# Vegeta2020/SE-SSD

Measured on NVIDIA H100. Metric: frames_per_sec, higher is better.
Workload: dtype f32

## Files before the change

include/sessd_b200.h:

```cpp
#ifndef SESSD_B200_H
#define SESSD_B200_H

#include <stddef.h>
#include <stdint.h>

#ifdef __cplusplus
extern "C" {
#endif

#define SESSD_OK 0
#define SESSD_EINVAL (-1)
#define SESSD_ECAPACITY (-2)
#define SESSD_EWORKSPACE (-3)

const char *sessd_version(void);
long long sessd_launch_count(void);

typedef struct {
    float voxel_size[3];
    float range_min[3];
    float range_max[3];
    int grid[3];
    int max_points;
    int max_voxels;
// ... 27 lines not shown

int sessd_strided_rulebook(const int *d_in_coors, const int *d_n_in, int max_in, sessd_grid in_grid,
                           int in_index_kind, const void *d_in_index, int in_hash_capacity,
                           const int ksize[3], const int stride[3], const int padding[3],
                           sessd_grid out_grid, void *d_out_bitmap , void *d_scan_scratch,
                           int *d_out_coors, int *d_n_out, int max_out, int *d_nbr, int *d_status, void *stream);

int sessd_tile_list_stride(int kvol);
int sessd_rulebook_tile_lists(const int *d_nbr, int kvol, const int *d_n_out, int max_out, void *d_tiles, void *stream);
size_t sessd_rulebook_pairs_workspace_bytes(int max_rows, int kvol);
int sessd_rulebook_pairs(const int *d_nbr, const int *d_n_out, int max_rows, int kvol, int *d_pairs_in,
                         int *d_pairs_out, int *d_pair_num, void *workspace, size_t workspace_bytes, void *stream);

int sessd_spconv_forward(const float *d_in_feat, int cin, const int *d_nbr, int kvol, const int *d_n_out,
                         int max_out, const float *d_weight, int cout, const float *d_scale, const float *d_shift,
                         int relu, float *d_out_feat, void *stream);

int sessd_sparse_to_dense(const float *d_feat, const int *d_coors, const int *d_n, int max_rows, int channels,
                          sessd_grid grid, float *d_out, void *stream);
int sessd_sparse_to_dense_indexed(const float *d_feat, int max_rows, const void *d_bitmap_index, int channels, sessd_grid grid,
                                  float *d_out, void *stream);

int sessd_spconv_forward_rows(const float *d_in_feat, int cin, const int *d_nbr, int kvol, const int *d_n_out, int max_out,
                              const float *d_weight, int cout, const float *d_scale, const float *d_shift, int relu,
                              float *d_out_feat, float *d_amax_out, void *stream);
int sessd_spconv_forward_rows_planes(const float *d_in_feat, int cin, const int *d_nbr, int kvol, const int *d_n_out, int max_out,
                                     const float *d_weight, int cout, const float *d_scale, const float *d_shift, int relu,
                                     const float *d_amax_in, float gain, float shift_max, float *d_out_feat, void *d_out_planes, int cpo,
                                     float *d_out_info, void *stream);
int sessd_spconv_forward_cg(const void *d_in_planes, int cp, int plane_rows, const float *d_in_info, const void *d_tiles, int kvol,
                            const int *d_n_out, int max_out, const void *d_weight_h2, int cout, const float *d_scale, const float *d_shift,
                            int relu, float gain, float shift_max, float *d_out_f32, void *d_out_planes, float *d_out_info, void *stream);
void sessd_set_sp_cg_deep(int on);
int sessd_absmax_rows(const float *d_feat, const int *d_n, int max_rows, int channels, float *d_amax, void *stream);

int sessd_rulebook_transpose(const int *d_nbr, int kvol, const int *d_n_out, int max_out, int max_in, int *d_nbr_t, void *stream);
int sessd_sparse_split_planes(const float *d_x, const int *d_n, int max_rows, int channels, float *d_info, void *d_planes, int cp, void *stream);
int sessd_dense_grad_gather(const float *d_grad, const int *d_coors, const int *d_n, int max_rows, int channels, sessd_grid grid,
                            float *d_out, void *stream);
int sessd_spconv_wgrad_items(int max_out, int kvol);
size_t sessd_spconv_wgrad_workspace_bytes(int max_out, int kvol, int cin, int cout);
int sessd_spconv_wgrad_rows(const float *d_in_feat, int cin, const float *d_gout, int cout, const void *d_tiles, int kvol,
                            const int *d_n_out, int max_out, float *d_gw, void *d_ws, size_t ws_bytes, void *stream);
int sessd_spconv_wgrad_cg(const void *d_in_planes, int cp, const float *d_in_info, const void *d_g_planes, int cout, const float *d_g_info,
                          const void *d_tiles, int kvol, const int *d_n_out, int max_out, float *d_gw, void *d_ws, size_t ws_bytes,
                          void *stream);

typedef struct {
    int batch, in_h, in_w, cin;
    int out_h, out_w, cout;
    int grid_h, grid_w;
    int in_stride;
    int out_stride, out_off_y, out_off_x;
    int ntaps;
    int tap_dy[16], tap_dx[16];
    int relu;
} sessd_conv_desc;

int sessd_bev_conv_p2(const void *d_in_planes, const float *d_in_info, const void *d_weight_h2, int cout_pad, const float *d_scale,
                      const float *d_shift, const float *d_residual, const float *d_resid_info, float gain, float shift_max,
                      float *d_out_f32, void *d_out_planes, float *d_out_info, const sessd_conv_desc *desc, const int *d_items,
                      void *stream);
int sessd_bev_deconv_p2(const void *d_in_planes, const float *d_in_info, const void *d_weight_h2, int cout_pad, const float *d_scale,
                        const float *d_shift, const float *d_residual, const float *d_resid_info, float gain, float shift_max,
                        float *d_out_f32, void *d_out_planes, float *d_out_info, int batch, int in_h, int in_w, int cin, int cout,
                        int relu, const int *d_items, void *stream);
// ... 169 lines not shown
```

se-ssd_b200/csrc/spconv_cg.cu:

```cuda
#include <cuda_fp16.h>

#include "tc_common.cuh"
#include "tile_lists.cuh"

namespace sessd {

constexpr int kCgBM = 128;
constexpr int kCgMaxK = 27;
constexpr int kCgProdWarps = 8;
constexpr int kCgMmaWarps = 8;
constexpr int kCgWeightWarp = kCgProdWarps + kCgMmaWarps;
constexpr int kCgThreads = (kCgWeightWarp + 1) * 32;

template <int CP, int COUT, int DEEP = 0>
struct CgCfg {
    static constexpr bool kWide = (CP == 64);
    static constexpr int kATile = (kWide ? 2 : 1) * kCgBM * 128;
    static constexpr int kBTile = (kWide ? 2 : 1) * COUT * 128;
    static constexpr int kStage = kATile + (kBTile + 1023) / 1024 * 1024;
    static constexpr int kStages = (kWide ? 2 : 4) * (DEEP ? 2 : 1);
    static constexpr int kMeta = kCgBM * kCgMaxK * 4  + kCgMaxK * 16  + 2 * COUT * 4  + 32 * 4  +
                                 33 * 4  + 32 * 4  + 3 * kStages * 8  + 24;
    static constexpr int kSmem = kStages * kStage + kMeta + 1024;
    static constexpr int kCPO = COUT > 32 ? 64 : 32;
};

struct CgArgs {
    const __half *planes;
    const float *in_info;
    const unsigned int *tiles;
    int tile_stride;
    const int *d_n_out;
    int kvol, max_out, relu;
    const float *scale, *shift;
    float gain, shift_max;
    float *out_f32;
    __half *out_planes;
    float *out_info;
};

__device__ __forceinline__ void cg_cp_async16(uint32_t smem_dst, const void *gsrc) {
    asm volatile("cp.async.cg.shared.global [%0], [%1], 16;\n" ::"r"(smem_dst), "l"(gsrc) : "memory");
}
__device__ __forceinline__ void cg_fence_proxy_async() { asm volatile("fence.proxy.async.shared::cta;\n" ::: "memory"); }
__device__ __forceinline__ void cg_sts_zero16(uint32_t saddr) {
    asm volatile("st.shared.v4.b32 [%0], {%1, %1, %1, %1};\n" ::"r"(saddr), "r"(0) : "memory");
}

template <int N>
__device__ __forceinline__ void cg_wgmma(float *d, uint64_t da, uint64_t db, uint32_t accumulate) {
    if constexpr (N == 32) wgmma_f16_n32(d, da, db, accumulate);
    else if constexpr (N == 64) wgmma_f16_n64(d, da, db, accumulate);
    else wgmma_f16_n128(d, da, db, accumulate);
}

template <int CP, int COUT, int DEEP>
__global__ void __launch_bounds__(kCgThreads, 1) spconv_cg_kernel(const __grid_constant__ CUtensorMap map_w, const CgArgs a) {
    using C = CgCfg<CP, COUT, DEEP>;
    const int n_out = min(*a.d_n_out, a.max_out);
    const int ntiles = (n_out + kCgBM - 1) / kCgBM;
    if ((int)blockIdx.x >= ntiles) return;
    const int kvol = a.kvol;
    if (threadIdx.x == kCgWeightWarp * 32) prefetch_tensormap(&map_w);

    extern __shared__ unsigned char smem_raw[];
    unsigned char *tiles = (unsigned char *)(((uintptr_t)smem_raw + 1023) & ~(uintptr_t)1023);
    uint32_t *s_list = (uint32_t *)(tiles + C::kStages * C::kStage);
    uint32_t *s_valid = s_list + kCgBM * kCgMaxK;
    float *s_scale = (float *)(s_valid + kCgMaxK * 4);
    float *s_shift = s_scale + COUT;
    int *s_cnt = (int *)(s_shift + COUT);
    int *s_klist = s_cnt + 32;
    int *s_nact = s_klist + 32;
    int *s_off = s_nact + 1;
    uint64_t *bars = (uint64_t *)(((uintptr_t)(s_off + 32) + 7) & ~(uintptr_t)7);
    uint64_t *full_a = bars, *full_b = bars + C::kStages, *empty = bars + 2 * C::kStages;

    const int tid = threadIdx.x, warp = tid >> 5, lane = tid & 31;
    const uint32_t tiles_u32 = smem_u32(tiles);

    if (tid == 0) {
        for (int s = 0; s < C::kStages; ++s) { mbar_init(&full_a[s], kCgProdWarps / C::kStages); mbar_init(&full_b[s], 1); mbar_init(&empty[s], kCgMmaWarps); }
        asm volatile("fence.mbarrier_init.release.cluster;\n" ::: "memory");
    }
    if (tid < COUT) {
        s_scale[tid] = __ldg(a.scale + tid);
        s_shift[tid] = a.shift ? __ldg(a.shift + tid) : 0.f;
    }
    for (int s = 0; s < C::kStages; ++s)
        for (int o = tid * 16; o < C::kATile; o += kCgThreads * 16) cg_sts_zero16(tiles_u32 + (uint32_t)(s * C::kStage + o));
    cg_fence_proxy_async();
    __syncthreads();

    const float amax_in = __ldg(a.in_info), s_in = __ldg(a.in_info + 1);
    const float inv_act = 1.f / s_in;
    const float s_out = pow2_scale_for_bound(amax_in * a.gain + a.shift_max);
    if (blockIdx.x == 0 && tid == 0 && a.out_info) a.out_info[1] = s_out;
    float vmax = 0.f;
    uint32_t dirty[4] = {0u, 0u, 0u, 0u};
    int st0 = 0;
    uint32_t ph0 = 0;

    for (int tile = blockIdx.x; tile < ntiles; tile += gridDim.x) {
        const int row0 = tile * kCgBM;
        const int rows = min(kCgBM, n_out - row0);
        {
            const unsigned int *rec = a.tiles + (size_t)tile * (size_t)a.tile_stride;
            const int c = (int)__ldg(rec + lane);
            unsigned int spec[4];
#pragma unroll
            for (int u = 0; u < 4; ++u) spec[u] = (tid + u * kCgThreads < kTlRows * kvol) ? __ldg(rec + kTlHeader + tid + u * kCgThreads) : 0u;
            const int incl = warp_incl_scan(c, lane);
            const int total = __shfl_sync(0xffffffffu, incl, 31);
            if (warp == 0) {
                s_cnt[lane] = c;
                s_off[lane] = incl - c;
                const unsigned int m = __ballot_sync(0xffffffffu, c > 0);
                if (c > 0) s_klist[__popc(m & ((1u << lane) - 1u))] = lane;
                if (lane == 0) *s_nact = __popc(m);
            }
            if (tid < kvol * 4) s_valid[tid] = __ldg(rec + kTlMask + tid);
#pragma unroll
            for (int u = 0; u < 4; ++u)
                if (tid + u * kCgThreads < total) s_list[tid + u * kCgThreads] = spec[u];
            for (int e = tid + 4 * kCgThreads; e < total; e += kCgThreads) s_list[e] = __ldg(rec + kTlHeader + e);
        }
        __syncthreads();
        const int nact = *s_nact;

        if (warp == kCgWeightWarp) {
            int s = st0;
            uint32_t ph = ph0;
            for (int j = 0; j < nact; ++j) {
                const int k = s_klist[j];
                mbar_wait(&empty[s], ph ^ 1u);
                if (elect_one()) {
                    mbar_expect_tx(&full_b[s], C::kBTile);
                    unsigned char *b_tile = tiles + s * C::kStage + C::kATile;
                    tma_load_4d(b_tile + C::kBTile / 2, &map_w, &full_b[s], 0, 0, 0, k);
                    tma_load_4d(b_tile, &map_w, &full_b[s], 0, 0, 1, k);
                }
                __syncwarp();
                if (++s == C::kStages) { s = 0; ph ^= 1u; }
            }
        } else if (warp >= kCgProdWarps) {
            const int cw = warp - kCgProdWarps, wg = cw >> 2, wq = cw & 3;
            constexpr int kAcc = COUT / 2;
            float acc[COUT];
#pragma unroll
            for (int i = 0; i < COUT; ++i) acc[i] = 0.f;
            const uint32_t a_rows = (uint32_t)(wg * 64 * 128);
            int s = st0;
            uint32_t ph = ph0;
            for (int j = 0; j < nact; ++j) {
                mbar_wait(&full_b[s], ph);
                mbar_wait(&full_a[s], ph);
                const uint32_t st = tiles_u32 + (uint32_t)(s * C::kStage);
                const uint64_t dA = kDescSw128Hi | desc_lo(st + a_rows);
                const uint32_t first = j != 0 ? 1u : 0u;
                wgmma_fence();
                if constexpr (C::kWide) {
                    const uint64_t dAl = dA + ((kCgBM * 128) >> 4);
                    const uint64_t dBl = kDescSw128Hi | desc_lo(st + C::kATile);
                    const uint64_t dBh = dBl + ((COUT * 128) >> 4);
#pragma unroll
                    for (int kk = 0; kk < 4; ++kk) cg_wgmma<2 * COUT>(acc, dA + 2 * kk, dBl + 2 * kk, first | (kk != 0));
#pragma unroll
                    for (int kk = 0; kk < 4; ++kk) cg_wgmma<COUT>(acc, dAl + 2 * kk, dBh + 2 * kk, 1u);
                } else {
                    const uint64_t dBl = kDescSw64Hi | desc_lo(st + C::kATile);
                    const uint64_t dBh = dBl + ((COUT * 64) >> 4);
#pragma unroll
                    for (int kk = 0; kk < 2; ++kk) cg_wgmma<2 * COUT>(acc, dA + 2 * kk, dBl + 2 * kk, first | (kk != 0));
#pragma unroll
                    for (int kk = 0; kk < 2; ++kk) cg_wgmma<COUT>(acc, dA + 4 + 2 * kk, dBh + 2 * kk, 1u);
                }
                wgmma_commit();
                wgmma_wait<0>();
                if (lane == 0) mbar_arrive(&empty[s]);
                if (++s == C::kStages) { s = 0; ph ^= 1u; }
            }
            wgmma_fence_regs<COUT>(acc);
#pragma unroll
            for (int i = 0; i < kAcc; ++i) acc[i] = acc[kAcc + i] + acc[i];
            const int q = lane & 3;
            const int r0 = wg * 64 + wq * 16 + (lane >> 2);
#pragma unroll
            for (int jb = 0; jb < COUT / 32; ++jb)
#pragma unroll
                for (int h = 0; h < 2; ++h) {
                    const int r = r0 + 8 * h;
                    const bool row_ok = r < rows;
                    const size_t orow = (size_t)(row0 + r);
                    float v[8], o[8];
                    quad_transpose8(acc + 16 * jb + 2 * h, q, v);
                    const int n = 32 * jb + 8 * q;
#pragma unroll
                    for (int t = 0; t < 8; t += 4) {
                        const float4 sc = *reinterpret_cast<const float4 *>(s_scale + n + t);
                        const float4 sh = *reinterpret_cast<const float4 *>(s_shift + n + t);
                        o[t] = fmaf(v[t] * inv_act, sc.x, sh.x);
                        o[t + 1] = fmaf(v[t + 1] * inv_act, sc.y, sh.y);
                        o[t + 2] = fmaf(v[t + 2] * inv_act, sc.z, sh.z);
                        o[t + 3] = fmaf(v[t + 3] * inv_act, sc.w, sh.w);
                    }
                    if (a.relu) {
#pragma unroll
                        for (int t = 0; t < 8; ++t) o[t] = fmaxf(o[t], 0.f);
                    }
                    if (row_ok) {
#pragma unroll
                        for (int t = 0; t < 8; ++t) vmax = fmaxf(vmax, fabsf(o[t]));
                    }
                    if (a.out_planes && row_ok) {
                        __align__(16) __half2 hi[4], lo[4];
#pragma unroll
                        for (int t = 0; t < 4; ++t) {
                            const float x0 = o[2 * t] * s_out, x1 = o[2 * t + 1] * s_out;
                            hi[t] = __floats2half2_rn(x0, x1);
                            const float2 f = __half22float2(hi[t]);
                            lo[t] = __floats2half2_rn(x0 - f.x, x1 - f.y);
                        }
                        __half *dst = a.out_planes + orow * (2 * C::kCPO) + n;
                        *reinterpret_cast<uint4 *>(dst) = *reinterpret_cast<const uint4 *>(hi);
                        *reinterpret_cast<uint4 *>(dst + C::kCPO) = *reinterpret_cast<const uint4 *>(lo);
                    }
                    if (a.out_f32) {
                        const bool up = q & 2;
                        float keep[4], recv[4];
#pragma unroll
                        for (int t = 0; t < 4; ++t) {
                            keep[t] = up ? o[4 + t] : o[t];
                            recv[t] = __shfl_xor_sync(0xFFFFFFFFu, up ? o[t] : o[4 + t], 2);
                        }
                        const float4 w_lo = up ? make_float4(recv[0], recv[1], recv[2], recv[3]) : make_float4(keep[0], keep[1], keep[2], keep[3]);
                        const float4 w_hi = up ? make_float4(keep[0], keep[1], keep[2], keep[3]) : make_float4(recv[0], recv[1], recv[2], recv[3]);
                        float *dst = a.out_f32 + orow * COUT + 32 * jb + 8 * (q & 1) + 4 * (q >> 1);
                        if (row_ok) {
                            *reinterpret_cast<float4 *>(dst) = w_lo;
                            *reinterpret_cast<float4 *>(dst + 16) = w_hi;
                        }
                    }
                }
        } else {
            constexpr int kGroupWarps = kCgProdWarps / C::kStages;
            constexpr int kGroupThreads = kGroupWarps * 32;
            constexpr int kOwnRows = kCgBM / kGroupWarps;
            constexpr int kOwnWords = kOwnRows / 32;
            constexpr int kLanesPerRow = C::kWide ? 16 : 8;
            constexpr int kRowsPerPass = kGroupThreads / kLanesPerRow;
            const int grp = warp / kGroupWarps, gw = warp % kGroupWarps;
            const int gtid = tid - grp * kGroupThreads;
            const int slot = gtid / kLanesPerRow;
            const int c = gtid % kLanesPerRow;
            const int half = c >> 3, cc = c & 7;
            const uint32_t a_base = tiles_u32 + (uint32_t)(grp * C::kStage);
            for (int j = (grp - st0 + C::kStages) % C::kStages; j < nact; j += C::kStages) {
                const uint32_t ph = ph0 ^ ((uint32_t)((st0 + j) / C::kStages) & 1u);
                const int k = s_klist[j];
                if (lane == 0) mbar_wait(&empty[grp], ph ^ 1u);
                __syncwarp();
#pragma unroll
                for (int w = 0; w < kOwnWords; ++w) {
                    const uint32_t vs = s_valid[k * 4 + gw * kOwnWords + w];
                    const uint32_t z = dirty[w] & ~vs;
                    dirty[w] = vs;
                    if (z) {
#pragma unroll
                        for (int q4 = 0; q4 < 8; ++q4) {
                            const int r32 = q4 * 4 + (lane >> 3);
                            if ((z >> r32) & 1u) {
                                const uint32_t dst = a_base + (uint32_t)((gw * kOwnRows + w * 32 + r32) * 128 + (lane & 7) * 16);
                                cg_sts_zero16(dst);
                                if constexpr (C::kWide) cg_sts_zero16(dst + kCgBM * 128);
                            }
                        }
                    }
                }
                const int n = s_cnt[k];
                const uint32_t *lst = s_list + s_off[k];
                auto copy_row = [&](uint32_t e) {
                    const uint32_t r = tl_tile_row(e);
                    const size_t src = (size_t)tl_in_row(e);
                    if constexpr (C::kWide)
                        cg_cp_async16(a_base + (uint32_t)half * (kCgBM * 128) + r * 128u + (((uint32_t)cc ^ (r & 7u)) << 4),
                                      a.planes + src * 128 + half * 64 + cc * 8);
                    else
                        cg_cp_async16(a_base + r * 128u + (((uint32_t)cc ^ (r & 7u)) << 4), a.planes + src * 64 + cc * 8);
                };
                int i = slot;
                for (; i + 3 * kRowsPerPass < n; i += 4 * kRowsPerPass) {
                    const uint32_t e0 = lst[i], e1 = lst[i + kRowsPerPass], e2 = lst[i + 2 * kRowsPerPass], e3 = lst[i + 3 * kRowsPerPass];
                    copy_row(e0); copy_row(e1); copy_row(e2); copy_row(e3);
                }
                for (; i < n; i += kRowsPerPass) copy_row(lst[i]);
                asm volatile("cp.async.wait_all;\n" ::: "memory");
                cg_fence_proxy_async();
                __syncwarp();
                if (lane == 0) mbar_arrive(&full_a[grp]);
            }
        }
        {
            const int adv = st0 + nact;
            ph0 ^= (uint32_t)(adv / C::kStages) & 1u;
            st0 = adv % C::kStages;
        }
        __syncthreads();
    }
    if (warp >= kCgProdWarps && warp < kCgWeightWarp && a.out_info) {
        const unsigned m = __reduce_max_sync(0xFFFFFFFFu, __float_as_uint(vmax));
        if (lane == 0 && m != 0u) atomicMax(reinterpret_cast<unsigned *>(a.out_info), m);
    }
}

static int g_cg_deep = 0;

template <int CP, int COUT, int DEEP>
static int launch_spconv_cg(const CgArgs &a, const void *w_h2, cudaStream_t st) {
    using C = CgCfg<CP, COUT, DEEP>;
    static bool attr_done = false;
    if (!attr_done) {
        cudaError_t e = cudaFuncSetAttribute(spconv_cg_kernel<CP, COUT, DEEP>, cudaFuncAttributeMaxDynamicSharedMemorySize, C::kSmem);
        if (e != cudaSuccess) return (int)e;
        attr_done = true;
    }
    CUtensorMap map_w;
    int rc;
    if (C::kWide) {
        const cuuint64_t dims[4] = {64, (cuuint64_t)COUT, 2, (cuuint64_t)a.kvol};
        const cuuint32_t box[4] = {64, (cuuint32_t)COUT, 1, 1};
        rc = encode_map_4d(&map_w, w_h2, dims, box, nullptr, CU_TENSOR_MAP_DATA_TYPE_FLOAT16, 2);
    } else {
        EncodeTiledFn enc = get_tensor_map_encoder();
        if (!enc) return SESSD_EINVAL;
        const cuuint64_t dims[4] = {32, (cuuint64_t)COUT, 2, (cuuint64_t)a.kvol};
        const cuuint64_t strides[3] = {64, (cuuint64_t)COUT * 64, (cuuint64_t)COUT * 128};
        const cuuint32_t box[4] = {32, (cuuint32_t)COUT, 1, 1};
        const cuuint32_t estr[4] = {1, 1, 1, 1};
        CUresult r = enc(&map_w, CU_TENSOR_MAP_DATA_TYPE_FLOAT16, 4, const_cast<void *>(w_h2), dims, strides, box, estr, CU_TENSOR_MAP_INTERLEAVE_NONE,
                         CU_TENSOR_MAP_SWIZZLE_64B, CU_TENSOR_MAP_L2_PROMOTION_L2_128B, CU_TENSOR_MAP_FLOAT_OOB_FILL_NONE);
        rc = r == CUDA_SUCCESS ? 0 : 700 + (int)r;
    }
    if (rc) return rc;
    static int num_sms = 0;
    if (!num_sms) {
        int dev = 0;
        SESSD_CUDA_TRY(cudaGetDevice(&dev));
        SESSD_CUDA_TRY(cudaDeviceGetAttribute(&num_sms, cudaDevAttrMultiProcessorCount, dev));
    }
    const int tiles = div_up(a.max_out, kCgBM);
    const int grid = tiles < num_sms ? tiles : num_sms;
    SESSD_LAUNCH((spconv_cg_kernel<CP, COUT, DEEP>), grid, kCgThreads, C::kSmem, st, map_w, a);
    return last_error();
}

}

using namespace sessd;

extern "C" void sessd_set_sp_cg_deep(int on) { sessd::g_cg_deep = on ? 1 : 0; }

extern "C" int sessd_spconv_forward_cg(const void *d_in_planes, int cp, int plane_rows, const float *d_in_info, const void *d_tiles, int kvol,
                                       const int *d_n_out, int max_out, const void *d_weight_h2, int cout, const float *d_scale,
                                       const float *d_shift, int relu, float gain, float shift_max, float *d_out_f32, void *d_out_planes,
                                       float *d_out_info, void *stream) {
    if (!d_in_planes || !d_in_info || !d_tiles || !d_n_out || !d_weight_h2 || !d_scale || (!d_out_f32 && !d_out_planes) || max_out < 1 ||
        kvol < 1 || kvol > kCgMaxK || plane_rows < 1 || plane_rows > (1 << 25))
        return SESSD_EINVAL;
    if (d_out_planes && !d_out_info) return SESSD_EINVAL;
    if (((uintptr_t)d_out_f32 | (uintptr_t)d_out_planes) & 15) return SESSD_EINVAL;
    CgArgs a;
    a.planes = (const __half *)d_in_planes; a.in_info = d_in_info; a.tiles = (const unsigned int *)d_tiles; a.tile_stride = tile_list_stride(kvol); a.d_n_out = d_n_out; a.kvol = kvol; a.max_out = max_out;
    a.relu = relu; a.scale = d_scale; a.shift = d_shift; a.gain = gain; a.shift_max = shift_max; a.out_f32 = d_out_f32;
    a.out_planes = (__half *)d_out_planes; a.out_info = d_out_info;
    cudaStream_t st = (cudaStream_t)stream;
#define SESSD_CG_CASE(CPV, CO) \
    if (cp == CPV && cout == CO) return g_cg_deep ? launch_spconv_cg<CPV, CO, 1>(a, d_weight_h2, st) : launch_spconv_cg<CPV, CO, 0>(a, d_weight_h2, st);
    SESSD_CG_CASE(32, 32)
    SESSD_CG_CASE(32, 64)
    SESSD_CG_CASE(64, 32)
    SESSD_CG_CASE(64, 64)
#undef SESSD_CG_CASE
    return SESSD_EINVAL;
}
```

se-ssd_b200/sessd_b200/_lib.py:

```python
import ctypes as C
import os

_HERE = os.path.dirname(os.path.abspath(__file__))
LIB_PATH = os.path.join(os.path.dirname(_HERE), "libsessd_b200.so")
LAB_PATH = os.path.join(os.path.dirname(_HERE), "libsessd_b200_lab.so")


class SessdError(RuntimeError):
    pass


class VoxelCfg(C.Structure):
    _fields_ = [("voxel_size", C.c_float * 3), ("range_min", C.c_float * 3), ("range_max", C.c_float * 3),
                ("grid", C.c_int * 3), ("max_points", C.c_int), ("max_voxels", C.c_int), ("num_feat", C.c_int)]


class Grid(C.Structure):
    _fields_ = [("batch", C.c_int), ("shape", C.c_int * 3)]


class ConvDesc(C.Structure):
    _fields_ = [("batch", C.c_int), ("in_h", C.c_int), ("in_w", C.c_int), ("cin", C.c_int),
                ("out_h", C.c_int), ("out_w", C.c_int), ("cout", C.c_int),
                ("grid_h", C.c_int), ("grid_w", C.c_int), ("in_stride", C.c_int),
# ... 8 lines not shown
                ("direction_offset", C.c_float), ("use_frustum", C.c_int)]


class KittiFrames(C.Structure):
    _fields_ = [("num_frames", C.c_int), ("gt_off", C.c_void_p), ("gt", C.c_void_p), ("gt_code", C.c_void_p),
                ("gt_occluded", C.c_void_p), ("dc_off", C.c_void_p), ("dc", C.c_void_p), ("dt_off", C.c_void_p),
                ("dt_cnt", C.c_void_p), ("dt", C.c_void_p), ("dt_code", C.c_void_p), ("ov_off", C.c_void_p)]


_vp, _i, _f, _sz, _ll = C.c_void_p, C.c_int, C.c_float, C.c_size_t, C.c_longlong
_I3 = C.POINTER(C.c_int)

SIGNATURES = {
    "sessd_version": (C.c_char_p, []),
    "sessd_launch_count": (_ll, []),
    "sessd_voxelize_workspace_bytes": (_sz, [_i, _i, C.POINTER(VoxelCfg)]),
    "sessd_voxelize": (_i, [_vp, _vp, _i, _i, C.POINTER(VoxelCfg), _vp, _vp, _vp, _vp, _vp, _vp, _sz, _vp]),
    "sessd_voxelize_host": (_i, [_vp, _i, C.POINTER(VoxelCfg), _vp, _vp, _vp]),
    "sessd_hash_bytes": (_sz, [_i, _I3]),
    "sessd_hash_build": (_i, [_vp, _vp, _i, Grid, _vp, _i, _vp]),
    "sessd_bitmap_words": (_sz, [Grid]),
    "sessd_scan_scratch_bytes": (_sz, [_sz]),
    "sessd_subm_rulebook": (_i, [_vp, _vp, _i, Grid, _I3, _i, _vp, _i, _vp, _vp]),
    "sessd_strided_rulebook": (_i, [_vp, _vp, _i, Grid, _i, _vp, _i, _I3, _I3, _I3, Grid, _vp, _vp, _vp, _vp, _i, _vp, _vp, _vp]),
    "sessd_tile_list_stride": (_i, [_i]),
    "sessd_rulebook_tile_lists": (_i, [_vp, _i, _vp, _i, _vp, _vp]),
    "sessd_rulebook_pairs_workspace_bytes": (_sz, [_i, _i]),
    "sessd_rulebook_pairs": (_i, [_vp, _vp, _i, _i, _vp, _vp, _vp, _vp, _sz, _vp]),
    "sessd_spconv_forward": (_i, [_vp, _i, _vp, _i, _vp, _i, _vp, _i, _vp, _vp, _i, _vp, _vp]),
    "sessd_spconv_forward_rows": (_i, [_vp, _i, _vp, _i, _vp, _i, _vp, _i, _vp, _vp, _i, _vp, _vp, _vp]),
    "sessd_spconv_forward_rows_planes": (_i, [_vp, _i, _vp, _i, _vp, _i, _vp, _i, _vp, _vp, _i, _vp, _f, _f, _vp, _vp, _i, _vp, _vp]),
    "sessd_spconv_forward_cg": (_i, [_vp, _i, _i, _vp, _vp, _i, _vp, _i, _vp, _i, _vp, _vp, _i, _f, _f, _vp, _vp, _vp, _vp]),
    "sessd_set_sp_cg_deep": (None, [_i]),
    "sessd_absmax_rows": (_i, [_vp, _vp, _i, _i, _vp, _vp]),
    "sessd_rulebook_transpose": (_i, [_vp, _i, _vp, _i, _i, _vp, _vp]),
    "sessd_sparse_split_planes": (_i, [_vp, _vp, _i, _i, _vp, _vp, _i, _vp]),
    "sessd_dense_grad_gather": (_i, [_vp, _vp, _vp, _i, _i, Grid, _vp, _vp]),
    "sessd_spconv_wgrad_items": (_i, [_i, _i]),
    "sessd_spconv_wgrad_workspace_bytes": (_sz, [_i, _i, _i, _i]),
    "sessd_spconv_wgrad_rows": (_i, [_vp, _i, _vp, _i, _vp, _i, _vp, _i, _vp, _vp, _sz, _vp]),
    "sessd_spconv_wgrad_cg": (_i, [_vp, _i, _vp, _vp, _i, _vp, _vp, _i, _vp, _i, _vp, _vp, _sz, _vp]),
    "sessd_sparse_to_dense_indexed": (_i, [_vp, _i, _vp, _i, Grid, _vp, _vp]),
    "sessd_sparse_to_dense": (_i, [_vp, _vp, _vp, _i, _i, Grid, _vp, _vp]),
    "sessd_bev_conv_p2": (_i, [_vp, _vp, _vp, _i, _vp, _vp, _vp, _vp, _f, _f, _vp, _vp, _vp, C.POINTER(ConvDesc), _vp, _vp]),
    "sessd_bev_deconv_p2": (_i, [_vp, _vp, _vp, _i, _vp, _vp, _vp, _vp, _f, _f, _vp, _vp, _vp, _i, _i, _i, _i, _i, _i, _vp, _vp]),
    "sessd_bev_skip_plan_words": (_ll, [_i, _i, _i, _I3]),
    "sessd_bev_skip_plan": (_i, [_vp, Grid, _vp, _vp]),
    "sessd_bev_skip_fill": (_i, [_vp, _vp, _vp, _i, _vp]),
    "sessd_bev_wgrad_items": (_i, [C.POINTER(ConvDesc)]),
    "sessd_bev_wgrad_workspace_bytes": (_sz, [C.POINTER(ConvDesc)]),
    "sessd_bev_wgrad": (_i, [_vp, _vp, _vp, _vp, C.POINTER(ConvDesc), _vp, _vp, _sz, _vp]),
    "sessd_bev_split_planes": (_i, [_vp, _ll, _vp, _vp, _vp]),
    "sessd_sparse_to_dense_planes": (_i, [_vp, _i, _vp, _i, Grid, _vp, _vp, _vp, _vp]),
    "sessd_ssfa_fuse_planes": (_i, [_vp, _vp, _vp, _vp, _f, _f, _f, _f, _i, _i, _vp, _vp, _vp, _vp, _vp, _vp]),
    "sessd_absmax": (_i, [_vp, C.c_longlong, _vp, _vp]),
    "sessd_postprocess_workspace_bytes": (_sz, [C.POINTER(PostCfg)]),
    "sessd_postprocess": (_i, [_vp, _vp, _vp, C.POINTER(PostCfg), _vp, _vp, _vp, _vp, _vp, _vp, _vp, _sz, _vp]),
    "sessd_postprocess_packed": (_i, [_vp, _vp, _vp, C.POINTER(PostCfg), _vp, _vp, _vp, _vp, _vp, _vp, _vp, _vp, _vp, _vp, _vp, _sz, _vp]),
    "sessd_rotate_nms_workspace_bytes": (_sz, [_i, _i]),
    "sessd_rotate_nms": (_i, [_vp, _vp, _vp, _i, _i, _i, _f, _i, _vp, _vp, _vp, _sz, _vp]),
    "sessd_boxes_overlap_bev": (_i, [_vp, _i, _vp, _i, _vp, _vp]),
    "sessd_boxes_aligned_overlap_bev": (_i, [_vp, _vp, _i, _vp, _vp]),
    "sessd_boxes_iou_bev": (_i, [_vp, _i, _vp, _i, _vp, _vp]),
    "sessd_boxes_iou3d": (_i, [_vp, _i, _vp, _i, _vp, _vp]),
    "sessd_nms_workspace_bytes": (_sz, [_i]),
    "sessd_nms_sorted": (_i, [_vp, _i, _f, _i, _vp, _vp, _vp, _sz, _vp]),
# ... 105 lines not shown
```

se-ssd_b200/sessd_b200/ops.py:

```python
import ctypes as C

import numpy as np
import torch

from . import _lib
from ._lib import ConvDesc, Grid, PostCfg, VoxelCfg, check, lib


def _p(t):
    return C.c_void_p(t.data_ptr()) if t is not None else C.c_void_p(0)


def _st():
    return C.c_void_p(torch.cuda.current_stream().cuda_stream)


def _cuda(t, dtype, name):
    if not (isinstance(t, torch.Tensor) and t.is_cuda and t.dtype == dtype and t.is_contiguous()):
        raise ValueError("%s must be a contiguous CUDA %s tensor" % (name, dtype))
    return t


def _i3(v):
    return (C.c_int * 3)(*[int(x) for x in v])
# ... 150 lines not shown
    return amax


def spconv_forward_rows_planes(in_feat, nbr, n_out, max_out, weight, scale, shift, relu, amax_in, gain, shift_max, out, out_planes, out_info):
    kvol, cin, cout = weight.shape
    check(lib.sessd_spconv_forward_rows_planes(_p(in_feat), int(cin), _p(nbr), int(kvol), _p(n_out), int(max_out), _p(weight), int(cout),
                                               _p(scale), _p(shift), int(bool(relu)), _p(amax_in), float(gain), float(shift_max), _p(out),
                                               _p(out_planes), int(out_planes.shape[1] // 2), _p(out_info), _st()),
          "sessd_spconv_forward_rows_planes")
    return out_planes


def alloc_tile_lists(max_out, kvol, device):
    return torch.zeros((-(-int(max_out) // 128), int(lib.sessd_tile_list_stride(int(kvol)))), dtype=torch.int32, device=device)


def rulebook_tile_lists(nbr, n_out, max_out, tiles):
    check(lib.sessd_rulebook_tile_lists(_p(nbr), int(nbr.shape[1]), _p(n_out), int(max_out), _p(tiles), _st()), "sessd_rulebook_tile_lists")
    return tiles


def spconv_forward_cg(in_planes, in_info, tiles, n_out, max_out, weight_h2, scale, shift, relu, gain, shift_max, out, out_planes, out_info):
    cp = in_planes.shape[1] // 2
    kvol = weight_h2.shape[0]
    cout = weight_h2.shape[2]
    check(lib.sessd_spconv_forward_cg(_p(in_planes), int(cp), int(in_planes.shape[0]), _p(in_info), _p(tiles), int(kvol), _p(n_out), int(max_out),
                                      _p(weight_h2), int(cout), _p(scale), _p(shift), int(bool(relu)), float(gain), float(shift_max), _p(out),
                                      _p(out_planes), _p(out_info), _st()), "sessd_spconv_forward_cg")
    return out if out is not None else out_planes


def set_sp_cg_deep(on):
    lib.sessd_set_sp_cg_deep(int(on))


def rulebook_transpose(nbr, n_out, max_out, max_in, nbr_t=None):
    kvol = int(nbr.shape[1])
    if nbr_t is None:
        nbr_t = torch.empty((int(max_in), kvol), dtype=torch.int32, device=nbr.device)
    check(lib.sessd_rulebook_transpose(_p(nbr), kvol, _p(n_out), int(max_out), int(max_in), _p(nbr_t), _st()), "sessd_rulebook_transpose")
    return nbr_t


def sparse_split_planes(x, n, max_rows, info, planes):
    check(lib.sessd_sparse_split_planes(_p(x), _p(n), int(max_rows), int(x.shape[1]), _p(info), _p(planes), int(planes.shape[1] // 2), _st()),
          "sessd_sparse_split_planes")
    return planes


def dense_grad_gather(grad, coors, n, max_rows, grid, channels, out=None):
    if out is None:
        out = torch.empty((int(max_rows), int(channels)), dtype=torch.float32, device=grad.device)
    check(lib.sessd_dense_grad_gather(_p(grad), _p(coors), _p(n), int(max_rows), int(channels), grid, _p(out), _st()), "sessd_dense_grad_gather")
    return out


def wgrad_items(max_out, kvol):
    return int(lib.sessd_spconv_wgrad_items(int(max_out), int(kvol)))


def wgrad_workspace(max_out, kvol, cin, cout, device):
    return torch.empty((int(lib.sessd_spconv_wgrad_workspace_bytes(int(max_out), int(kvol), int(cin), int(cout))),), dtype=torch.uint8,
                       device=device)


def spconv_wgrad_rows(in_feat, gout, tiles, n_out, max_out, kvol, gw=None, ws=None):
# ... 626 lines not shown
```

Baseline: 1466.

## Restructure sparse conv kernel for two CTAs per SM with register rebalancing

Drops the dedicated weight-loading warp and has producer group leaders issue the TMA weight loads. Producer warps drop from 8 to 4, and setmaxnreg splits registers between producer and MMA warps. Launch bounds move to two blocks per SM and the grid is sized from the queried occupancy. The goal is more concurrent tiles per SM to hide gather and wgmma latency, at the cost of fewer gather warps, register limits and tighter shared memory.

```diff
diff --git a/include/sessd_b200.h b/include/sessd_b200.h
--- a/include/sessd_b200.h
+++ b/include/sessd_b200.h
@@ -83,6 +83,7 @@
                             const int *d_n_out, int max_out, const void *d_weight_h2, int cout, const float *d_scale, const float *d_shift,
                             int relu, float gain, float shift_max, float *d_out_f32, void *d_out_planes, float *d_out_info, void *stream);
 void sessd_set_sp_cg_deep(int on);
+int sessd_spconv_cg_blocks_per_sm(int cp, int cout, int deep);
 int sessd_absmax_rows(const float *d_feat, const int *d_n, int max_rows, int channels, float *d_amax, void *stream);
 
 int sessd_rulebook_transpose(const int *d_nbr, int kvol, const int *d_n_out, int max_out, int max_in, int *d_nbr_t, void *stream);
diff --git a/se-ssd_b200/csrc/spconv_cg.cu b/se-ssd_b200/csrc/spconv_cg.cu
--- a/se-ssd_b200/csrc/spconv_cg.cu
+++ b/se-ssd_b200/csrc/spconv_cg.cu
@@ -7,10 +7,10 @@
 
 constexpr int kCgBM = 128;
 constexpr int kCgMaxK = 27;
-constexpr int kCgProdWarps = 8;
+constexpr int kCgProdWarps = 4;
 constexpr int kCgMmaWarps = 8;
-constexpr int kCgWeightWarp = kCgProdWarps + kCgMmaWarps;
-constexpr int kCgThreads = (kCgWeightWarp + 1) * 32;
+constexpr int kCgThreads = (kCgProdWarps + kCgMmaWarps) * 32;
+constexpr int kCgRegsProducer = 48, kCgRegsConsumer = 96;
 
 template <int CP, int COUT, int DEEP = 0>
 struct CgCfg {
@@ -19,6 +19,9 @@
     static constexpr int kBTile = (kWide ? 2 : 1) * COUT * 128;
     static constexpr int kStage = kATile + (kBTile + 1023) / 1024 * 1024;
     static constexpr int kStages = (kWide ? 2 : 4) * (DEEP ? 2 : 1);
+    static constexpr int kGroups = kStages < kCgProdWarps ? kStages : kCgProdWarps;
+    static constexpr int kGroupWarps = kCgProdWarps / kGroups;
+    static constexpr int kGroupStages = kStages / kGroups;
     static constexpr int kMeta = kCgBM * kCgMaxK * 4  + kCgMaxK * 16  + 2 * COUT * 4  + 32 * 4  +
                                  33 * 4  + 32 * 4  + 3 * kStages * 8  + 24;
     static constexpr int kSmem = kStages * kStage + kMeta + 1024;
@@ -49,19 +52,21 @@
 
 template <int N>
 __device__ __forceinline__ void cg_wgmma(float *d, uint64_t da, uint64_t db, uint32_t accumulate) {
+    static_assert(N == 32 || N == 64, "COUT is 32 or 64");
     if constexpr (N == 32) wgmma_f16_n32(d, da, db, accumulate);
-    else if constexpr (N == 64) wgmma_f16_n64(d, da, db, accumulate);
-    else wgmma_f16_n128(d, da, db, accumulate);
+    else wgmma_f16_n64(d, da, db, accumulate);
 }
 
 template <int CP, int COUT, int DEEP>
-__global__ void __launch_bounds__(kCgThreads, 1) spconv_cg_kernel(const __grid_constant__ CUtensorMap map_w, const CgArgs a) {
+__global__ void __launch_bounds__(kCgThreads, 2) spconv_cg_kernel(const __grid_constant__ CUtensorMap map_w, const CgArgs a) {
     using C = CgCfg<CP, COUT, DEEP>;
+    static_assert(DEEP || C::kSmem <= 113 * 1024, "two CTAs per SM: 228 KB of shared memory less 1 KB reserved per CTA");
+    static_assert(kCgProdWarps * 32 * kCgRegsProducer + kCgMmaWarps * 32 * kCgRegsConsumer <= kCgThreads * 80, "setmaxnreg budget");
     const int n_out = min(*a.d_n_out, a.max_out);
     const int ntiles = (n_out + kCgBM - 1) / kCgBM;
     if ((int)blockIdx.x >= ntiles) return;
     const int kvol = a.kvol;
-    if (threadIdx.x == kCgWeightWarp * 32) prefetch_tensormap(&map_w);
+    if (threadIdx.x == 0) prefetch_tensormap(&map_w);
 
     extern __shared__ unsigned char smem_raw[];
     unsigned char *tiles = (unsigned char *)(((uintptr_t)smem_raw + 1023) & ~(uintptr_t)1023);
@@ -80,7 +85,11 @@
     const uint32_t tiles_u32 = smem_u32(tiles);
 
     if (tid == 0) {
-        for (int s = 0; s < C::kStages; ++s) { mbar_init(&full_a[s], kCgProdWarps / C::kStages); mbar_init(&full_b[s], 1); mbar_init(&empty[s], kCgMmaWarps); }
+        for (int s = 0; s < C::kStages; ++s) {
+            mbar_init(&full_a[s], C::kGroupWarps);
+            mbar_init(&full_b[s], 1);
+            mbar_init(&empty[s], kCgMmaWarps);
+        }
         asm volatile("fence.mbarrier_init.release.cluster;\n" ::: "memory");
     }
     if (tid < COUT) {
@@ -92,179 +101,78 @@
     cg_fence_proxy_async();
     __syncthreads();
 
-    const float amax_in = __ldg(a.in_info), s_in = __ldg(a.in_info + 1);
-    const float inv_act = 1.f / s_in;
-    const float s_out = pow2_scale_for_bound(amax_in * a.gain + a.shift_max);
-    if (blockIdx.x == 0 && tid == 0 && a.out_info) a.out_info[1] = s_out;
-    float vmax = 0.f;
-    uint32_t dirty[4] = {0u, 0u, 0u, 0u};
+    auto load_lists = [&](int tile) {
+        const unsigned int *rec = a.tiles + (size_t)tile * (size_t)a.tile_stride;
+        const int c = (int)__ldg(rec + lane);
+        unsigned int spec[4];
+#pragma unroll
+        for (int u = 0; u < 4; ++u) spec[u] = (tid + u * kCgThreads < kTlRows * kvol) ? __ldg(rec + kTlHeader + tid + u * kCgThreads) : 0u;
+        const int incl = warp_incl_scan(c, lane);
+        const int total = __shfl_sync(0xffffffffu, incl, 31);
+        if (warp == 0) {
+            s_cnt[lane] = c;
+            s_off[lane] = incl - c;
+            const unsigned int m = __ballot_sync(0xffffffffu, c > 0);
+            if (c > 0) s_klist[__popc(m & ((1u << lane) - 1u))] = lane;
+            if (lane == 0) *s_nact = __popc(m);
+        }
+        if (tid < kvol * 4) s_valid[tid] = __ldg(rec + kTlMask + tid);
+#pragma unroll
+        for (int u = 0; u < 4; ++u)
+            if (tid + u * kCgThreads < total) s_list[tid + u * kCgThreads] = spec[u];
+        for (int e = tid + 4 * kCgThreads; e < total; e += kCgThreads) s_list[e] = __ldg(rec + kTlHeader + e);
+    };
     int st0 = 0;
     uint32_t ph0 = 0;
-
-    for (int tile = blockIdx.x; tile < ntiles; tile += gridDim.x) {
-        const int row0 = tile * kCgBM;
-        const int rows = min(kCgBM, n_out - row0);
-        {
-            const unsigned int *rec = a.tiles + (size_t)tile * (size_t)a.tile_stride;
-            const int c = (int)__ldg(rec + lane);
-            unsigned int spec[4];
-#pragma unroll
-            for (int u = 0; u < 4; ++u) spec[u] = (tid + u * kCgThreads < kTlRows * kvol) ? __ldg(rec + kTlHeader + tid + u * kCgThreads) : 0u;
-            const int incl = warp_incl_scan(c, lane);
-            const int total = __shfl_sync(0xffffffffu, incl, 31);
-            if (warp == 0) {
-                s_cnt[lane] = c;
-                s_off[lane] = incl - c;
-                const unsigned int m = __ballot_sync(0xffffffffu, c > 0);
-                if (c > 0) s_klist[__popc(m & ((1u << lane) - 1u))] = lane;
-                if (lane == 0) *s_nact = __popc(m);
-            }
-            if (tid < kvol * 4) s_valid[tid] = __ldg(rec + kTlMask + tid);
-#pragma unroll
-            for (int u = 0; u < 4; ++u)
-                if (tid + u * kCgThreads < total) s_list[tid + u * kCgThreads] = spec[u];
-            for (int e = tid + 4 * kCgThreads; e < total; e += kCgThreads) s_list[e] = __ldg(rec + kTlHeader + e);
-        }
-        __syncthreads();
-        const int nact = *s_nact;
-
-        if (warp == kCgWeightWarp) {
-            int s = st0;
-            uint32_t ph = ph0;
-            for (int j = 0; j < nact; ++j) {
+    auto advance_ring = [&](int nact) {
+        const int adv = st0 + nact;
+        ph0 ^= (uint32_t)(adv / C::kStages) & 1u;
+        st0 = adv % C::kStages;
+    };
+
+    if (warp < kCgProdWarps) {
+        setmaxnreg_dec<kCgRegsProducer>();
+        constexpr int kGroups = C::kGroups, kGroupWarps = C::kGroupWarps, kGroupStages = C::kGroupStages;
+        constexpr int kGroupThreads = kGroupWarps * 32;
+        constexpr int kOwnRows = kCgBM / kGroupWarps;
+        constexpr int kOwnWords = kOwnRows / 32;
+        constexpr int kLanesPerRow = C::kWide ? 16 : 8;
+        constexpr int kRowsPerPass = kGroupThreads / kLanesPerRow;
+        const int grp = warp / kGroupWarps, gw = warp % kGroupWarps;
+        const int gtid = tid - grp * kGroupThreads;
+        const int slot = gtid / kLanesPerRow;
+        const int c = gtid % kLanesPerRow;
+        const int half = c >> 3, cc = c & 7;
+        uint32_t dirty[kGroupStages][kOwnWords];
+#pragma unroll
+        for (int g = 0; g < kGroupStages; ++g)
+#pragma unroll
+            for (int w = 0; w < kOwnWords; ++w) dirty[g][w] = 0u;
+        for (int tile = blockIdx.x; tile < ntiles; tile += gridDim.x) {
+            load_lists(tile);
+            __syncthreads();
+            const int nact = *s_nact;
+            for (int j = (grp - st0 % kGroups + kGroups) % kGroups; j < nact; j += kGroups) {
+                const int pos = st0 + j;
+                const int s = pos % C::kStages;
+                const uint32_t ph = ph0 ^ ((uint32_t)(pos / C::kStages) & 1u);
                 const int k = s_klist[j];
-                mbar_wait(&empty[s], ph ^ 1u);
-                if (elect_one()) {
-                    mbar_expect_tx(&full_b[s], C::kBTile);
-                    unsigned char *b_tile = tiles + s * C::kStage + C::kATile;
-                    tma_load_4d(b_tile + C::kBTile / 2, &map_w, &full_b[s], 0, 0, 0, k);
-                    tma_load_4d(b_tile, &map_w, &full_b[s], 0, 0, 1, k);
-                }
-                __syncwarp();
-                if (++s == C::kStages) { s = 0; ph ^= 1u; }
-            }
-        } else if (warp >= kCgProdWarps) {
-            const int cw = warp - kCgProdWarps, wg = cw >> 2, wq = cw & 3;
-            constexpr int kAcc = COUT / 2;
-            float acc[COUT];
-#pragma unroll
-            for (int i = 0; i < COUT; ++i) acc[i] = 0.f;
-            const uint32_t a_rows = (uint32_t)(wg * 64 * 128);
-            int s = st0;
-            uint32_t ph = ph0;
-            for (int j = 0; j < nact; ++j) {
-                mbar_wait(&full_b[s], ph);
-                mbar_wait(&full_a[s], ph);
-                const uint32_t st = tiles_u32 + (uint32_t)(s * C::kStage);
-                const uint64_t dA = kDescSw128Hi | desc_lo(st + a_rows);
-                const uint32_t first = j != 0 ? 1u : 0u;
-                wgmma_fence();
-                if constexpr (C::kWide) {
-                    const uint64_t dAl = dA + ((kCgBM * 128) >> 4);
-                    const uint64_t dBl = kDescSw128Hi | desc_lo(st + C::kATile);
-                    const uint64_t dBh = dBl + ((COUT * 128) >> 4);
-#pragma unroll
-                    for (int kk = 0; kk < 4; ++kk) cg_wgmma<2 * COUT>(acc, dA + 2 * kk, dBl + 2 * kk, first | (kk != 0));
-#pragma unroll
-                    for (int kk = 0; kk < 4; ++kk) cg_wgmma<COUT>(acc, dAl + 2 * kk, dBh + 2 * kk, 1u);
-                } else {
-                    const uint64_t dBl = kDescSw64Hi | desc_lo(st + C::kATile);
-                    const uint64_t dBh = dBl + ((COUT * 64) >> 4);
-#pragma unroll
-                    for (int kk = 0; kk < 2; ++kk) cg_wgmma<2 * COUT>(acc, dA + 2 * kk, dBl + 2 * kk, first | (kk != 0));
-#pragma unroll
-                    for (int kk = 0; kk < 2; ++kk) cg_wgmma<COUT>(acc, dA + 4 + 2 * kk, dBh + 2 * kk, 1u);
-                }
-                wgmma_commit();
-                wgmma_wait<0>();
-                if (lane == 0) mbar_arrive(&empty[s]);
-                if (++s == C::kStages) { s = 0; ph ^= 1u; }
-            }
-            wgmma_fence_regs<COUT>(acc);
-#pragma unroll
-            for (int i = 0; i < kAcc; ++i) acc[i] = acc[kAcc + i] + acc[i];
-            const int q = lane & 3;
-            const int r0 = wg * 64 + wq * 16 + (lane >> 2);
-#pragma unroll
-            for (int jb = 0; jb < COUT / 32; ++jb)
-#pragma unroll
-                for (int h = 0; h < 2; ++h) {
-                    const int r = r0 + 8 * h;
-                    const bool row_ok = r < rows;
-                    const size_t orow = (size_t)(row0 + r);
-                    float v[8], o[8];
-                    quad_transpose8(acc + 16 * jb + 2 * h, q, v);
-                    const int n = 32 * jb + 8 * q;
-#pragma unroll
-                    for (int t = 0; t < 8; t += 4) {
-                        const float4 sc = *reinterpret_cast<const float4 *>(s_scale + n + t);
-                        const float4 sh = *reinterpret_cast<const float4 *>(s_shift + n + t);
-                        o[t] = fmaf(v[t] * inv_act, sc.x, sh.x);
-                        o[t + 1] = fmaf(v[t + 1] * inv_act, sc.y, sh.y);
-                        o[t + 2] = fmaf(v[t + 2] * inv_act, sc.z, sh.z);
-                        o[t + 3] = fmaf(v[t + 3] * inv_act, sc.w, sh.w);
-                    }
-                    if (a.relu) {
-#pragma unroll
-                        for (int t = 0; t < 8; ++t) o[t] = fmaxf(o[t], 0.f);
-                    }
-                    if (row_ok) {
-#pragma unroll
-                        for (int t = 0; t < 8; ++t) vmax = fmaxf(vmax, fabsf(o[t]));
-                    }
-                    if (a.out_planes && row_ok) {
-                        __align__(16) __half2 hi[4], lo[4];
-#pragma unroll
-                        for (int t = 0; t < 4; ++t) {
-                            const float x0 = o[2 * t] * s_out, x1 = o[2 * t + 1] * s_out;
-                            hi[t] = __floats2half2_rn(x0, x1);
-                            const float2 f = __half22float2(hi[t]);
-                            lo[t] = __floats2half2_rn(x0 - f.x, x1 - f.y);
-                        }
-                        __half *dst = a.out_planes + orow * (2 * C::kCPO) + n;
-                        *reinterpret_cast<uint4 *>(dst) = *reinterpret_cast<const uint4 *>(hi);
-                        *reinterpret_cast<uint4 *>(dst + C::kCPO) = *reinterpret_cast<const uint4 *>(lo);
-                    }
-                    if (a.out_f32) {
-                        const bool up = q & 2;
-                        float keep[4], recv[4];
-#pragma unroll
-                        for (int t = 0; t < 4; ++t) {
-                            keep[t] = up ? o[4 + t] : o[t];
-                            recv[t] = __shfl_xor_sync(0xFFFFFFFFu, up ? o[t] : o[4 + t], 2);
-                        }
-                        const float4 w_lo = up ? make_float4(recv[0], recv[1], recv[2], recv[3]) : make_float4(keep[0], keep[1], keep[2], keep[3]);
-                        const float4 w_hi = up ? make_float4(keep[0], keep[1], keep[2], keep[3]) : make_float4(recv[0], recv[1], recv[2], recv[3]);
-                        float *dst = a.out_f32 + orow * COUT + 32 * jb + 8 * (q & 1) + 4 * (q >> 1);
-                        if (row_ok) {
-                            *reinterpret_cast<float4 *>(dst) = w_lo;
-                            *reinterpret_cast<float4 *>(dst + 16) = w_hi;
-                        }
-                    }
-                }
-        } else {
-            constexpr int kGroupWarps = kCgProdWarps / C::kStages;
-            constexpr int kGroupThreads = kGroupWarps * 32;
-            constexpr int kOwnRows = kCgBM / kGroupWarps;
-            constexpr int kOwnWords = kOwnRows / 32;
-            constexpr int kLanesPerRow = C::kWide ? 16 : 8;
-            constexpr int kRowsPerPass = kGroupThreads / kLanesPerRow;
-            const int grp = warp / kGroupWarps, gw = warp % kGroupWarps;
-            const int gtid = tid - grp * kGroupThreads;
-            const int slot = gtid / kLanesPerRow;
-            const int c = gtid % kLanesPerRow;
-            const int half = c >> 3, cc = c & 7;
-            const uint32_t a_base = tiles_u32 + (uint32_t)(grp * C::kStage);
-            for (int j = (grp - st0 + C::kStages) % C::kStages; j < nact; j += C::kStages) {
-                const uint32_t ph = ph0 ^ ((uint32_t)((st0 + j) / C::kStages) & 1u);
-                const int k = s_klist[j];
-                if (lane == 0) mbar_wait(&empty[grp], ph ^ 1u);
+                const uint32_t a_base = tiles_u32 + (uint32_t)(s * C::kStage);
+                if (lane == 0) {
+                    mbar_wait<true>(&empty[s], ph ^ 1u);
+                    if (gw == 0) {
+                        mbar_expect_tx(&full_b[s], C::kBTile);
+                        unsigned char *b_tile = tiles + s * C::kStage + C::kATile;
+                        tma_load_4d(b_tile + C::kBTile / 2, &map_w, &full_b[s], 0, 0, 0, k);
+                        tma_load_4d(b_tile, &map_w, &full_b[s], 0, 0, 1, k);
+                    }
+                }
                 __syncwarp();
 #pragma unroll
                 for (int w = 0; w < kOwnWords; ++w) {
                     const uint32_t vs = s_valid[k * 4 + gw * kOwnWords + w];
-                    const uint32_t z = dirty[w] & ~vs;
-                    dirty[w] = vs;
+                    const uint32_t z = dirty[0][w] & ~vs;
+                    dirty[0][w] = vs;
                     if (z) {
 #pragma unroll
                         for (int q4 = 0; q4 < 8; ++q4) {
@@ -297,33 +205,170 @@
                 asm volatile("cp.async.wait_all;\n" ::: "memory");
                 cg_fence_proxy_async();
                 __syncwarp();
-                if (lane == 0) mbar_arrive(&full_a[grp]);
+                if (lane == 0) mbar_arrive(&full_a[s]);
+                if constexpr (kGroupStages > 1) {
+#pragma unroll
+                    for (int w = 0; w < kOwnWords; ++w) {
+                        const uint32_t d = dirty[0][w];
+#pragma unroll
+                        for (int g = 0; g + 1 < kGroupStages; ++g) dirty[g][w] = dirty[g + 1][w];
+                        dirty[kGroupStages - 1][w] = d;
+                    }
+                }
             }
+            advance_ring(nact);
+            __syncthreads();
         }
-        {
-            const int adv = st0 + nact;
-            ph0 ^= (uint32_t)(adv / C::kStages) & 1u;
-            st0 = adv % C::kStages;
+    } else {
+        setmaxnreg_inc<kCgRegsConsumer>();
+        const int cw = warp - kCgProdWarps, wg = cw >> 2, wq = cw & 3;
+        constexpr int kAcc = COUT / 2;
+        const float amax_in = __ldg(a.in_info), s_in = __ldg(a.in_info + 1);
+        const float inv_act = 1.f / s_in;
+        const float s_out = pow2_scale_for_bound(amax_in * a.gain + a.shift_max);
+        if (blockIdx.x == 0 && cw == 0 && lane == 0 && a.out_info) a.out_info[1] = s_out;
+        float vmax = 0.f;
+        const uint32_t a_rows = (uint32_t)(wg * 64 * 128);
+        for (int tile = blockIdx.x; tile < ntiles; tile += gridDim.x) {
+            load_lists(tile);
+            __syncthreads();
+            const int nact = *s_nact;
+            const int row0 = tile * kCgBM;
+            const int rows = min(kCgBM, n_out - row0);
+            float acc[kAcc], acc_main[kAcc];
+#pragma unroll
+            for (int i = 0; i < kAcc; ++i) acc[i] = acc_main[i] = 0.f;
+            int s = st0;
+            uint32_t ph = ph0;
+            for (int j = 0; j < nact; ++j) {
+                mbar_wait<true>(&full_b[s], ph);
+                mbar_wait<true>(&full_a[s], ph);
+                const uint32_t st = tiles_u32 + (uint32_t)(s * C::kStage);
+                const uint64_t dA = kDescSw128Hi | desc_lo(st + a_rows);
+                const uint32_t first = j != 0 ? 1u : 0u;
+                wgmma_fence();
+                if constexpr (C::kWide) {
+                    const uint64_t dAl = dA + ((kCgBM * 128) >> 4);
+                    const uint64_t dBl = kDescSw128Hi | desc_lo(st + C::kATile);
+                    const uint64_t dBh = dBl + ((COUT * 128) >> 4);
+#pragma unroll
+                    for (int kk = 0; kk < 4; ++kk) {
+                        cg_wgmma<COUT>(acc, dA + 2 * kk, dBl + 2 * kk, first | (kk != 0));
+                        cg_wgmma<COUT>(acc_main, dA + 2 * kk, dBh + 2 * kk, first | (kk != 0));
+                    }
+#pragma unroll
+                    for (int kk = 0; kk < 4; ++kk) cg_wgmma<COUT>(acc, dAl + 2 * kk, dBh + 2 * kk, 1u);
+                } else {
+                    const uint64_t dBl = kDescSw64Hi | desc_lo(st + C::kATile);
+                    const uint64_t dBh = dBl + ((COUT * 64) >> 4);
+#pragma unroll
+                    for (int kk = 0; kk < 2; ++kk) {
+                        cg_wgmma<COUT>(acc, dA + 2 * kk, dBl + 2 * kk, first | (kk != 0));
+                        cg_wgmma<COUT>(acc_main, dA + 2 * kk, dBh + 2 * kk, first | (kk != 0));
+                    }
+#pragma unroll
+                    for (int kk = 0; kk < 2; ++kk) cg_wgmma<COUT>(acc, dA + 4 + 2 * kk, dBh + 2 * kk, 1u);
+                }
+                wgmma_commit();
+                wgmma_wait<0>();
+                if (lane == 0) mbar_arrive(&empty[s]);
+                if (++s == C::kStages) { s = 0; ph ^= 1u; }
+            }
+            wgmma_fence_regs<kAcc>(acc);
+            wgmma_fence_regs<kAcc>(acc_main);
+#pragma unroll
+            for (int i = 0; i < kAcc; ++i) acc[i] = acc_main[i] + acc[i];
+            const int q = lane & 3;
+            const int r0 = wg * 64 + wq * 16 + (lane >> 2);
+#pragma unroll
+            for (int jb = 0; jb < COUT / 32; ++jb)
+#pragma unroll
+                for (int h = 0; h < 2; ++h) {
+                    const int r = r0 + 8 * h;
+                    const bool row_ok = r < rows;
+                    const size_t orow = (size_t)(row0 + r);
+                    float v[8], o[8];
+                    quad_transpose8(acc + 16 * jb + 2 * h, q, v);
+                    const int n = 32 * jb + 8 * q;
+#pragma unroll
+                    for (int t = 0; t < 8; t += 4) {
+                        const float4 sc = *reinterpret_cast<const float4 *>(s_scale + n + t);
+                        const float4 sh = *reinterpret_cast<const float4 *>(s_shift + n + t);
+                        o[t] = fmaf(v[t] * inv_act, sc.x, sh.x);
+                        o[t + 1] = fmaf(v[t + 1] * inv_act, sc.y, sh.y);
+                        o[t + 2] = fmaf(v[t + 2] * inv_act, sc.z, sh.z);
+                        o[t + 3] = fmaf(v[t + 3] * inv_act, sc.w, sh.w);
+                    }
+                    if (a.relu) {
+#pragma unroll
+                        for (int t = 0; t < 8; ++t) o[t] = fmaxf(o[t], 0.f);
+                    }
+                    if (row_ok) {
+#pragma unroll
+                        for (int t = 0; t < 8; ++t) vmax = fmaxf(vmax, fabsf(o[t]));
+                    }
+                    if (a.out_planes && row_ok) {
+                        __align__(16) __half2 hi[4], lo[4];
+#pragma unroll
+                        for (int t = 0; t < 4; ++t) {
+                            const float x0 = o[2 * t] * s_out, x1 = o[2 * t + 1] * s_out;
+                            hi[t] = __floats2half2_rn(x0, x1);
+                            const float2 f = __half22float2(hi[t]);
+                            lo[t] = __floats2half2_rn(x0 - f.x, x1 - f.y);
+                        }
+                        __half *dst = a.out_planes + orow * (2 * C::kCPO) + n;
+                        *reinterpret_cast<uint4 *>(dst) = *reinterpret_cast<const uint4 *>(hi);
+                        *reinterpret_cast<uint4 *>(dst + C::kCPO) = *reinterpret_cast<const uint4 *>(lo);
+                    }
+                    if (a.out_f32) {
+                        const bool up = q & 2;
+                        float keep[4], recv[4];
+#pragma unroll
+                        for (int t = 0; t < 4; ++t) {
+                            keep[t] = up ? o[4 + t] : o[t];
+                            recv[t] = __shfl_xor_sync(0xFFFFFFFFu, up ? o[t] : o[4 + t], 2);
+                        }
+                        const float4 w_lo = up ? make_float4(recv[0], recv[1], recv[2], recv[3]) : make_float4(keep[0], keep[1], keep[2], keep[3]);
+                        const float4 w_hi = up ? make_float4(keep[0], keep[1], keep[2], keep[3]) : make_float4(recv[0], recv[1], recv[2], recv[3]);
+                        float *dst = a.out_f32 + orow * COUT + 32 * jb + 8 * (q & 1) + 4 * (q >> 1);
+                        if (row_ok) {
+                            *reinterpret_cast<float4 *>(dst) = w_lo;
+                            *reinterpret_cast<float4 *>(dst + 16) = w_hi;
+                        }
+                    }
+                }
+            advance_ring(nact);
+            __syncthreads();
         }
-        __syncthreads();
-    }
-    if (warp >= kCgProdWarps && warp < kCgWeightWarp && a.out_info) {
-        const unsigned m = __reduce_max_sync(0xFFFFFFFFu, __float_as_uint(vmax));
-        if (lane == 0 && m != 0u) atomicMax(reinterpret_cast<unsigned *>(a.out_info), m);
+        if (a.out_info) {
+            const unsigned m = __reduce_max_sync(0xFFFFFFFFu, __float_as_uint(vmax));
+            if (lane == 0 && m != 0u) atomicMax(reinterpret_cast<unsigned *>(a.out_info), m);
+        }
     }
 }
 
 static int g_cg_deep = 0;
+
+template <int CP, int COUT, int DEEP>
+static cudaError_t cg_blocks_per_sm(int *blocks) {
+    using C = CgCfg<CP, COUT, DEEP>;
+    static int cached = 0;
+    if (!cached) {
+        cudaError_t e = cudaFuncSetAttribute(spconv_cg_kernel<CP, COUT, DEEP>, cudaFuncAttributeMaxDynamicSharedMemorySize, C::kSmem);
+        if (e == cudaSuccess)
+            e = cudaOccupancyMaxActiveBlocksPerMultiprocessor(&cached, spconv_cg_kernel<CP, COUT, DEEP>, kCgThreads, C::kSmem);
+        if (e != cudaSuccess) { cached = 0; return e; }
+        if (!cached) return cudaErrorInvalidConfiguration;
+    }
+    *blocks = cached;
+    return cudaSuccess;
+}
 
 template <int CP, int COUT, int DEEP>
 static int launch_spconv_cg(const CgArgs &a, const void *w_h2, cudaStream_t st) {
     using C = CgCfg<CP, COUT, DEEP>;
-    static bool attr_done = false;
-    if (!attr_done) {
-        cudaError_t e = cudaFuncSetAttribute(spconv_cg_kernel<CP, COUT, DEEP>, cudaFuncAttributeMaxDynamicSharedMemorySize, C::kSmem);
-        if (e != cudaSuccess) return (int)e;
-        attr_done = true;
-    }
+    int blocks_per_sm = 0;
+    SESSD_CUDA_TRY((cg_blocks_per_sm<CP, COUT, DEEP>(&blocks_per_sm)));
     CUtensorMap map_w;
     int rc;
     if (C::kWide) {
@@ -349,7 +394,7 @@
         SESSD_CUDA_TRY(cudaDeviceGetAttribute(&num_sms, cudaDevAttrMultiProcessorCount, dev));
     }
     const int tiles = div_up(a.max_out, kCgBM);
-    const int grid = tiles < num_sms ? tiles : num_sms;
+    const int grid = tiles < blocks_per_sm * num_sms ? tiles : blocks_per_sm * num_sms;
     SESSD_LAUNCH((spconv_cg_kernel<CP, COUT, DEEP>), grid, kCgThreads, C::kSmem, st, map_w, a);
     return last_error();
 }
@@ -359,6 +404,21 @@
 using namespace sessd;
 
 extern "C" void sessd_set_sp_cg_deep(int on) { sessd::g_cg_deep = on ? 1 : 0; }
+
+template <int CP, int COUT>
+static int cg_blocks_per_sm_or_error(int deep) {
+    int blocks = 0;
+    const cudaError_t e = deep ? cg_blocks_per_sm<CP, COUT, 1>(&blocks) : cg_blocks_per_sm<CP, COUT, 0>(&blocks);
+    return e == cudaSuccess ? blocks : -(int)e;
+}
+
+extern "C" int sessd_spconv_cg_blocks_per_sm(int cp, int cout, int deep) {
+    if (cp == 32 && cout == 32) return cg_blocks_per_sm_or_error<32, 32>(deep);
+    if (cp == 32 && cout == 64) return cg_blocks_per_sm_or_error<32, 64>(deep);
+    if (cp == 64 && cout == 32) return cg_blocks_per_sm_or_error<64, 32>(deep);
+    if (cp == 64 && cout == 64) return cg_blocks_per_sm_or_error<64, 64>(deep);
+    return SESSD_EINVAL;
+}
 
 extern "C" int sessd_spconv_forward_cg(const void *d_in_planes, int cp, int plane_rows, const float *d_in_info, const void *d_tiles, int kvol,
                                        const int *d_n_out, int max_out, const void *d_weight_h2, int cout, const float *d_scale,
diff --git a/se-ssd_b200/sessd_b200/_lib.py b/se-ssd_b200/sessd_b200/_lib.py
--- a/se-ssd_b200/sessd_b200/_lib.py
+++ b/se-ssd_b200/sessd_b200/_lib.py
@@ -64,6 +64,7 @@
     "sessd_spconv_forward_rows_planes": (_i, [_vp, _i, _vp, _i, _vp, _i, _vp, _i, _vp, _vp, _i, _vp, _f, _f, _vp, _vp, _i, _vp, _vp]),
     "sessd_spconv_forward_cg": (_i, [_vp, _i, _i, _vp, _vp, _i, _vp, _i, _vp, _i, _vp, _vp, _i, _f, _f, _vp, _vp, _vp, _vp]),
     "sessd_set_sp_cg_deep": (None, [_i]),
+    "sessd_spconv_cg_blocks_per_sm": (_i, [_i, _i, _i]),
     "sessd_absmax_rows": (_i, [_vp, _vp, _i, _i, _vp, _vp]),
     "sessd_rulebook_transpose": (_i, [_vp, _i, _vp, _i, _i, _vp, _vp]),
     "sessd_sparse_split_planes": (_i, [_vp, _vp, _i, _i, _vp, _vp, _i, _vp]),
diff --git a/se-ssd_b200/sessd_b200/ops.py b/se-ssd_b200/sessd_b200/ops.py
--- a/se-ssd_b200/sessd_b200/ops.py
+++ b/se-ssd_b200/sessd_b200/ops.py
@@ -206,6 +206,12 @@
 
 def set_sp_cg_deep(on):
     lib.sessd_set_sp_cg_deep(int(on))
+
+
+def spconv_cg_blocks_per_sm(cp, cout, deep=0):
+    n = int(lib.sessd_spconv_cg_blocks_per_sm(int(cp), int(cout), int(deep)))
+    check(min(n, 0), "sessd_spconv_cg_blocks_per_sm")
+    return n
 
 
 def rulebook_transpose(nbr, n_out, max_out, max_in, nbr_t=None):
```

New measurement: 1545 (median of 6 runs). +5.4%, better.
